# asmuth-archive/libsmatrix

Hardware: NVIDIA B200
Metric: incr_mops_c2 (higher is better)
Workload: dtype u32

## Files before the change

include/smatrix_b200.h:

```cpp
#ifndef SMATRIX_B200_H
#define SMATRIX_B200_H

#include "smatrix.h"

#ifdef __cplusplus
extern "C" {
#endif

smatrix_t* smatrix_b200_open(const char* fname, int device);
smatrix_t* smatrix_b200_open_arena(const char* fname, int device, size_t arena_bytes);

int   smatrix_b200_snapshot(smatrix_t* self);

int      smatrix_b200_snap_extent(smatrix_t* self, uint64_t* rows, uint64_t* bytes);
uint64_t smatrix_b200_snap_rows_base(uint64_t total_rows);
int      smatrix_b200_snap_layout(int fd, uint64_t total_rows, uint64_t total_bytes);
int      smatrix_b200_snap_write(smatrix_t* self, int fd, uint64_t byte_base, uint64_t first_entry);
int      smatrix_b200_snap_commit(const char* tmp, const char* fname);
typedef struct smx_loader_s smx_loader_t;
smx_loader_t* smatrix_b200_load_begin(smatrix_t* self, int fd, int share, int shares);
int  smatrix_b200_load_next(smx_loader_t* ld, const uint32_t** d_xs, const uint32_t** d_ys, const uint32_t** d_vs,
                            size_t* n_ops, const uint32_t** d_keys, const uint32_t** d_logs, size_t* n_rows);
void smatrix_b200_load_end(smx_loader_t* ld);
void smatrix_b200_load_fixup(smatrix_t* self, const uint32_t* d_keys, const uint32_t* d_logs, size_t n);
// ... 2 lines not shown
void* smatrix_b200_stream(smatrix_t* self);
void  smatrix_b200_sync(smatrix_t* self);

void  smatrix_b200_timer_start(smatrix_t* self);
float smatrix_b200_timer_stop_ms(smatrix_t* self);

enum {
  SMX_STAT_ROWS = 0,
  SMX_STAT_NNZ = 1,
  SMX_STAT_DIR_CAP = 2,
  SMX_STAT_SLAB_BYTES = 3,
  SMX_STAT_DEVICE_BYTES = 4,
  SMX_STAT_LAUNCHES = 5,
  SMX_STAT_ROUNDS = 6,
  SMX_STAT_ROW_GROWS = 7,
  SMX_STAT_DIR_GROWS = 8,
  SMX_STAT_KERNEL_NS = 9,
  SMX_STAT_NS_PARTITION = 10, SMX_STAT_NS_UPSERT = 11, SMX_STAT_NS_GROW_PLAN = 12,
  SMX_STAT_NS_SLAB = 13, SMX_STAT_NS_MIGRATE = 14, SMX_STAT_NS_DIR = 15,
  SMX_STAT_VALUE_SUM = 16,
  SMX_STAT_LIVE_BUCKET_BYTES = 17,
  SMX_STAT_FREE_BYTES = 18,
  SMX_STAT_RECYCLED = 19,
  SMX_STAT_H2D_BYTES = 20,
  SMX_STAT_D2H_BYTES = 21,
  SMX_STAT_BUCKET_BYTES = 22,
  SMX_STAT_SPILLED = 23,
  SMX_STAT_SLICED_GETS = 24,
  SMX_STAT_WIDE_CHUNKS = 25,
  SMX_STAT_NS_ALLOC = 26,
  SMX_STAT_ALLOCS = 27,
  SMX_STAT_TOPK_BIG = 28,
  SMX_STAT_TOPK_PASSES = 29,
  SMX_STAT_REC_BIG = 30
};
uint64_t smatrix_b200_stat(smatrix_t* self, int which);

void smatrix_b200_set_kernel_timing(smatrix_t* self, int on);

void smatrix_b200_set_get_slices(smatrix_t* self, int mode);

void* smatrix_b200_host_alloc(size_t bytes);
void  smatrix_b200_host_free(void* p);

void* smatrix_b200_dev_alloc(smatrix_t* self, size_t bytes);
void  smatrix_b200_dev_free(smatrix_t* self, void* p);
void  smatrix_b200_memcpy(smatrix_t* self, void* dst, const void* src, size_t bytes);
void  smatrix_b200_memset0(smatrix_t* self, void* d_dst, size_t bytes);

void smatrix_b200_gen_c2_ops(smatrix_t* self, uint64_t seed, uint64_t first, size_t count,
                             uint32_t rows, uint32_t ycols, uint32_t* d_xs, uint32_t* d_ys);
void smatrix_b200_gen_c2_queries(smatrix_t* self, uint64_t seed_get, uint64_t seed_build,
                                 uint64_t first, size_t count, uint64_t n_build, uint32_t rows,
                                 uint32_t ycols, uint32_t* d_xs, uint32_t* d_ys);

void smatrix_b200_gen_c3_ops(smatrix_t* self, uint64_t seed, uint64_t first, size_t count,
                             const uint64_t* d_thr, uint32_t items, uint32_t* d_xs, uint32_t* d_ys);
void smatrix_b200_gen_c3_queries(smatrix_t* self, uint64_t seed_get, uint64_t seed_build, uint64_t first,
                                 size_t count, uint64_t n_build, const uint64_t* d_thr, uint32_t items,
                                 uint32_t* d_xs, uint32_t* d_ys);
void smatrix_b200_gen_c4_lens(smatrix_t* self, uint64_t seed, uint64_t first, size_t count,
                              const uint64_t* d_thr, uint32_t kmax, uint32_t* d_lens);
void smatrix_b200_gen_c4_ops(smatrix_t* self, uint64_t seed, uint64_t first, size_t count,
                             const uint64_t* d_offs, uint32_t rows, uint32_t* d_xs, uint32_t* d_ys,
                             uint32_t* d_vs);

double smatrix_b200_probe_random_read(smatrix_t* self, size_t footprint_bytes, size_t accesses, int width);
// ... 47 lines not shown
```

libsmatrix_b200/binding.py:

```python
from __future__ import annotations

import ctypes as C
import os

HERE = os.path.dirname(os.path.abspath(__file__))
DEFAULT_SO = os.environ.get("SMATRIX_B200_LIB") or os.path.join(HERE, "lib", "libsmatrix_b200.so")

u32p = C.POINTER(C.c_uint32)
u64p = C.POINTER(C.c_uint64)

PROTOTYPES = {
    "smatrix_open": (C.c_void_p, [C.c_char_p]),
    "smatrix_close": (None, [C.c_void_p]),
    "smatrix_get": (C.c_uint32, [C.c_void_p, C.c_uint32, C.c_uint32]),
    "smatrix_set": (C.c_uint32, [C.c_void_p, C.c_uint32, C.c_uint32, C.c_uint32]),
    "smatrix_incr": (C.c_uint32, [C.c_void_p, C.c_uint32, C.c_uint32, C.c_uint32]),
    "smatrix_decr": (C.c_uint32, [C.c_void_p, C.c_uint32, C.c_uint32, C.c_uint32]),
    "smatrix_rowlen": (C.c_uint32, [C.c_void_p, C.c_uint32]),
    "smatrix_getrow": (C.c_uint32, [C.c_void_p, C.c_uint32, C.c_void_p, C.c_size_t]),
    "smatrix_incr_batch": (None, [C.c_void_p, C.c_void_p, C.c_void_p, C.c_void_p, C.c_size_t]),
    "smatrix_decr_batch": (None, [C.c_void_p, C.c_void_p, C.c_void_p, C.c_void_p, C.c_size_t]),
    "smatrix_set_batch": (None, [C.c_void_p, C.c_void_p, C.c_void_p, C.c_void_p, C.c_size_t]),
    "smatrix_incr_batch_out": (None, [C.c_void_p, C.c_void_p, C.c_void_p, C.c_void_p, C.c_size_t, C.c_void_p]),
    "smatrix_decr_batch_out": (None, [C.c_void_p, C.c_void_p, C.c_void_p, C.c_void_p, C.c_size_t, C.c_void_p]),
# ... 86 lines not shown
    "smatrix_b200_shard_close": (None, [C.c_void_p]),
    "smatrix_b200_shard_local": (C.c_void_p, [C.c_void_p]),
    "smatrix_b200_shard_rank": (C.c_int, [C.c_void_p]),
    "smatrix_b200_shard_world": (C.c_int, [C.c_void_p]),
    "smatrix_b200_shard_reserve": (None, [C.c_void_p, C.c_size_t, C.c_size_t]),
    "smatrix_b200_shard_incr_batch": (None, [C.c_void_p, C.c_void_p, C.c_void_p, C.c_void_p, C.c_size_t, C.c_int]),
    "smatrix_b200_shard_decr_batch": (None, [C.c_void_p, C.c_void_p, C.c_void_p, C.c_void_p, C.c_size_t, C.c_int]),
    "smatrix_b200_shard_set_batch": (None, [C.c_void_p, C.c_void_p, C.c_void_p, C.c_void_p, C.c_size_t]),
    "smatrix_b200_shard_incr_batch_out": (None, [C.c_void_p, C.c_void_p, C.c_void_p, C.c_void_p, C.c_size_t, C.c_void_p]),
    "smatrix_b200_shard_decr_batch_out": (None, [C.c_void_p, C.c_void_p, C.c_void_p, C.c_void_p, C.c_size_t, C.c_void_p]),
    "smatrix_b200_shard_set_batch_out": (None, [C.c_void_p, C.c_void_p, C.c_void_p, C.c_void_p, C.c_size_t, C.c_void_p]),
    "smatrix_b200_shard_get_batch": (None, [C.c_void_p, C.c_void_p, C.c_void_p, C.c_size_t, C.c_void_p]),
    "smatrix_b200_shard_rowlen_batch": (None, [C.c_void_p, C.c_void_p, C.c_size_t, C.c_void_p]),
    "smatrix_b200_shard_cf_neighbors_batch": (C.c_uint64, [C.c_void_p, C.c_void_p, C.c_size_t, C.c_void_p, C.c_void_p,
                                                          C.c_void_p, C.c_uint64]),
    "smatrix_b200_shard_cf_topk_batch": (None, [C.c_void_p, C.c_void_p, C.c_size_t, C.c_uint32, C.c_void_p,
                                                C.c_void_p, C.c_void_p]),
    "smatrix_b200_shard_cf_recommend_batch": (None, [C.c_void_p, C.c_void_p, C.c_void_p, C.c_size_t, C.c_uint32,
                                                     C.c_void_p, C.c_void_p, C.c_void_p]),
    "smatrix_b200_shard_getrow_batch": (C.c_uint64, [C.c_void_p, C.c_void_p, C.c_size_t, C.c_void_p, C.c_void_p,
                                                    C.c_uint64]),
    "smatrix_b200_shard_stat": (C.c_uint64, [C.c_void_p, C.c_int]),
    "smatrix_b200_shard_stat_reset": (None, [C.c_void_p]),
    "smatrix_b200_shard_barrier": (None, [C.c_void_p]),
    "smatrix_b200_shard_sum": (C.c_uint64, [C.c_void_p, C.c_uint64]),
    "smatrix_b200_shard_max": (C.c_uint64, [C.c_void_p, C.c_uint64]),
})

STAT = {"rows": 0, "nnz": 1, "dir_cap": 2, "slab_bytes": 3, "device_bytes": 4, "launches": 5,
        "rounds": 6, "row_grows": 7, "dir_grows": 8, "kernel_ns": 9, "ns_partition": 10, "ns_upsert": 11,
        "ns_grow_plan": 12, "ns_slab": 13, "ns_migrate": 14, "ns_dir": 15, "value_sum": 16,
        "live_bucket_bytes": 17, "free_bytes": 18, "recycled": 19, "h2d_bytes": 20, "d2h_bytes": 21, "bucket_bytes": 22, "spilled": 23,
        "sliced_gets": 24, "wide_chunks": 25, "ns_alloc": 26, "allocs": 27,
        "topk_big": 28, "topk_passes": 29, "rec_big": 30}

_cache: dict[str, C.CDLL] = {}


def load(path: str | None = None) -> C.CDLL:
    path = os.path.abspath(path or DEFAULT_SO)
    lib = _cache.get(path)
    if lib is None:
        if not os.path.exists(path):
            raise ImportError(
                f"{path} not found: build the CUDA library first "
                "(python -m libsmatrix_b200.build). There is no CPU fallback.")
        lib = C.CDLL(path)
        for name, (res, args) in PROTOTYPES.items():
            fn = getattr(lib, name)
            fn.restype = res
            fn.argtypes = args
        _cache[path] = lib
    return lib
```

libsmatrix_b200/csrc/smx_host.c:

```c
#define _GNU_SOURCE
#include <cuda_runtime_api.h>
#include <pthread.h>
#include <stdarg.h>
#include <stdio.h>
#include <stdlib.h>
#include <string.h>
#include <time.h>
#include <errno.h>
#include <fcntl.h>
#include <sys/stat.h>
#include <sys/types.h>
#include <unistd.h>

#include "../../include/smatrix.h"
#include "../../include/smatrix_b200.h"
#include "../../include/smatrix_batch.h"
#include "smx_internal.h"

#define SMX_DIR_LOG_DEFAULT 20u
#define SMX_CHUNK_DEFAULT (1u << 26)
#define SMX_STAGE_MAX (1u << 23)
#define SMX_SEG_MIN ((size_t)64 << 20)
#define SMX_SEG_MAX ((size_t)16 << 30)
#define SMX_MAX_ROUNDS 128
// ... 74 lines not shown
    smx_dbuf_t rows;
    smx_dbuf_t host_out;
    smx_dbuf_t spill;
    smx_dbuf_t bo_addr[2], bo_idx[2], bo_seg, bo_tiles, bo_out, bo_sort;
    smx_dbuf_t tk_ctl;
    smx_dbuf_t tk_off;
    smx_dbuf_t tk_big;
    smx_dbuf_t tk_cids, tk_cscores;
    smx_dbuf_t tk_ids, tk_scores;
    smx_dbuf_t rc_in, rc_pos, rc_ctl, rc_items, rc_sort, rc_tids, rc_tscores, rc_red, rc_rids, rc_rscores;
    smx_dbuf_t rc_big, rc_keys, rc_vals, rc_flags;
    smx_dbuf_t ld_raw, ld_tiles, ld_cnt, ld_off, ld_ops, ld_fix;
  } db;
  uint32_t topk_pairs;
  uint64_t n_topk_big, n_topk_passes;
  uint64_t n_rec_big;

  unsigned long long* free_ptr[SMX_CLASSES];
  uint32_t free_cap[SMX_CLASSES];
  int debug;
  int migrate_tiles;
  uint32_t spill_cap;
  uint64_t n_spilled;
  int recycle;
  int presize;
  int get_slices;
  int get_flags;
  uint32_t get_slice_min;
  uint64_t n_sliced_gets;
  uint64_t n_wide_chunks;
  double alloc_ns;
  uint64_t n_allocs;

  uint64_t n_launches, n_rounds, n_row_grows, n_dir_grows, n_recycled;
  uint64_t bucket_bytes;
  uint64_t h2d_bytes, d2h_bytes;
  double phase_ns[8];
  int timing;
  cudaEvent_t ev0, ev1, t_start, t_stop;
  double kernel_ns;
  int preagg;
  char* fname;
  uint32_t* snap_keys;
  uint64_t snap_rows;
  uint64_t* snap_hoff;
  uint32_t* snap_hkeys;
};

static void smx_die(const char* fmt, ...) {
  va_list ap;
  printf("libsmatrix error: ");
  va_start(ap, fmt);
  vprintf(fmt, ap);
  va_end(ap);
  printf("\n");
  fflush(stdout);
  abort();
}
#define CK(call)                                                                        \
  do {                                                                                  \
    cudaError_t e_ = (call);                                                            \
    if (e_ != cudaSuccess) smx_die("%s failed: %s (%s:%d)", #call, cudaGetErrorString(e_), \
                                   __FILE__, __LINE__);                                 \
  } while (0)

static uint32_t env_u32(const char* name, uint32_t dflt) {
  const char* v = getenv(name);
// ... 319 lines not shown
  if (!s->dir_in_arena) CK(cudaFree(s->dir));
  else slab_give_back(s, (char*)s->dir, (size_t)s->dir_cap * sizeof(smx_row_t));
  s->dir = nd;
  s->dir_in_arena = in_arena;
  s->dir_cap = new_cap;
  s->n_dir_grows++;
  s->phase_ns[PH_DIR] += now_ns() - t0;
  return 1;
}

static void zero_round_counters(smatrix_t* s) {
  CK(cudaMemsetAsync(&s->d_ctl->n_defer, 0,
                     offsetof(smx_ctl_t, scratch) - offsetof(smx_ctl_t, n_defer), s->stream));
}

static void run_pass(smatrix_t* s, smx_ops_t ops, int op, int pass, const uint32_t* list, uint32_t m) {
  int flip = 0;
  uint32_t prev_defer = 0xFFFFFFFFu;
  for (int round = 0; m > 0; round++) {
    if (round >= SMX_MAX_ROUNDS) smx_die("update pass does not converge (%u ops left)", m);
    double t0 = now_ns();
    const uint64_t used_before = s->h_ctl->dir_used;
    zero_round_counters(s);
    s->lists.defer_out = s->defer[flip];
    timed_begin(s);
    smx_launch_upsert(s->stream, view_of(s), ops, s->lists, op, pass, list, m, s->preagg);
    timed_end(s);
    s->n_launches++;
    s->n_rounds++;
    read_ctl(s);
    timed_collect(s);
    s->phase_ns[PH_UPSERT] += now_ns() - t0;
    const smx_ctl_t c = *s->h_ctl;
    if (c.n_grow) grow_rows(s, c.n_grow);
    if (c.n_defer == 0) break;
    if (c.n_dirfull) {
      const uint64_t accepted = (uint64_t)m - c.n_defer;
      const uint64_t created = c.dir_used > used_before ? c.dir_used - used_before : 0;
      double ratio = accepted ? (double)created / (double)accepted : 1.0;
      if (ratio > 1.0) ratio = 1.0;
      if (ratio < 0.05) ratio = 0.05;
      uint64_t need = 4 * (c.dir_used + (uint64_t)(ratio * (double)c.n_dirfull));
      uint64_t cap = pow2_at_least(need);
      if (cap < s->dir_cap * 2) cap = s->dir_cap * 2;
      if (cap > s->dir_cap * 64) cap = s->dir_cap * 64;
      resize_dir(s, cap, 0);
    } else if (!c.n_grow && c.n_defer >= prev_defer) {
      smx_die("update pass made no progress (%u ops deferred)", c.n_defer);
    }
    prev_defer = c.n_defer;
    list = s->defer[flip];
    m = c.n_defer;
    flip ^= 1;
  }
}

static void maybe_shrink_dir(smatrix_t* s) {
  const uint64_t used = s->h_ctl->dir_used;
  uint64_t fit = pow2_at_least(4 * (used ? used : 1));
  const uint64_t floor_cap = 1ull << s->dir_log_min;
  if (fit < floor_cap) fit = floor_cap;
  if (fit * 4 <= s->dir_cap && fit > s->shrink_refused) resize_dir(s, fit, 1);
}

static void slice_geometry(const smatrix_t* s, uint32_t* parts_log, uint32_t* shift) {
  uint32_t dir_log = 0;
// ... 1541 lines not shown
      CK(cudaMemsetAsync(&s->d_ctl->scratch, 0, 8, s->stream));
      CK(cudaMemsetAsync(d_cnt, 0, 4, s->stream));
      smx_launch_sum_values(s->stream, view_of(s), big, d_cnt);
      copy_d2h(s, &s->h_small->n_big_sums, d_cnt, 4, s->stream);
      CK(cudaStreamSynchronize(s->stream));
      smx_launch_sum_values_big(s->stream, view_of(s), big, s->h_small->n_big_sums);
      s->n_launches += 2;
      read_ctl(s);
      r = s->h_ctl->scratch;
      break;
    }
    case SMX_STAT_LIVE_BUCKET_BYTES:
      CK(cudaMemsetAsync(&s->d_ctl->scratch, 0, 8, s->stream));
      smx_launch_live_bytes(s->stream, view_of(s));
      s->n_launches++;
      read_ctl(s);
      r = s->h_ctl->scratch;
      break;
    case SMX_STAT_FREE_BYTES:
      read_ctl(s);
      for (uint32_t c = SMX_MIN_SLAB_LOG; c < SMX_CLASSES; c++)
        if (s->h_ctl->free_cnt[c] > 0) r += (uint64_t)s->h_ctl->free_cnt[c] * (8ull << c);
      break;
    case SMX_STAT_RECYCLED: r = s->n_recycled; break;
    case SMX_STAT_BUCKET_BYTES: r = s->bucket_bytes; break;
    case SMX_STAT_SPILLED: r = s->n_spilled; break;
    case SMX_STAT_SLICED_GETS: r = s->n_sliced_gets; break;
    case SMX_STAT_WIDE_CHUNKS: r = s->n_wide_chunks; break;
    case SMX_STAT_NS_ALLOC: r = (uint64_t)s->alloc_ns; break;
    case SMX_STAT_ALLOCS: r = s->n_allocs; break;
    case SMX_STAT_TOPK_BIG: r = s->n_topk_big; break;
    case SMX_STAT_TOPK_PASSES: r = s->n_topk_passes; break;
    case SMX_STAT_REC_BIG: r = s->n_rec_big; break;
    case SMX_STAT_H2D_BYTES: r = s->h2d_bytes; break;
    case SMX_STAT_D2H_BYTES: r = s->d2h_bytes; break;
    case SMX_STAT_DIR_CAP: r = s->dir_cap; break;
    case SMX_STAT_SLAB_BYTES: r = s->slab_bytes; break;
    case SMX_STAT_DEVICE_BYTES: {
      r = s->seg_bytes + s->dir_cap * sizeof(smx_row_t) + (uint64_t)s->list_cap * (6 * 4 + sizeof(smx_plan_t)) +
          (uint64_t)s->stage_cap * 24 + (uint64_t)s->addrs_cap * 8 + (uint64_t)s->part_cap * 16;
      const smx_dbuf_t* db = (const smx_dbuf_t*)&s->db;
      for (size_t b = 0; b < sizeof s->db / sizeof *db; b++) r += db[b].bytes;
      break;
    }
    case SMX_STAT_LAUNCHES: r = s->n_launches; break;
    case SMX_STAT_ROUNDS: r = s->n_rounds; break;
    case SMX_STAT_ROW_GROWS: r = s->n_row_grows; break;
    case SMX_STAT_DIR_GROWS: r = s->n_dir_grows; break;
    case SMX_STAT_KERNEL_NS: r = (uint64_t)s->kernel_ns; break;
    case SMX_STAT_NS_PARTITION: r = (uint64_t)s->phase_ns[PH_PARTITION]; break;
    case SMX_STAT_NS_UPSERT: r = (uint64_t)s->phase_ns[PH_UPSERT]; break;
    case SMX_STAT_NS_GROW_PLAN: r = (uint64_t)s->phase_ns[PH_GROW_PLAN]; break;
    case SMX_STAT_NS_SLAB: r = (uint64_t)s->phase_ns[PH_SLAB]; break;
    case SMX_STAT_NS_MIGRATE: r = (uint64_t)s->phase_ns[PH_MIGRATE]; break;
    case SMX_STAT_NS_DIR: r = (uint64_t)s->phase_ns[PH_DIR]; break;
    default: break;
  }
  leave(s);
  return r;
}

void* smatrix_b200_host_alloc(size_t bytes) {
  void* p = NULL;
  if (cudaHostAlloc(&p, bytes ? bytes : 1, cudaHostAllocDefault) != cudaSuccess) return NULL;
  return p;
}
// ... 310 lines not shown
```

libsmatrix_b200/csrc/smx_internal.h:

```cpp
#ifndef SMX_INTERNAL_H
#define SMX_INTERNAL_H

#include <stddef.h>
#include <stdint.h>

#ifdef __cplusplus
extern "C" {
#endif

#define SMX_META_CAPLOG 0x3Fu
#define SMX_META_USED   0x100u
#define SMX_META_ZC     0x200u
#define SMX_META_D      0x400u
#define SMX_META_SLOG_SHIFT 16
#define SMX_META_SLOG   (0x1Fu << SMX_META_SLOG_SHIFT)
#define SMX_META_T0P    0x800u
#define SMX_META_GROW   0x1000u
#define SMX_INLINE_LOG  2u
#define SMX_MIN_SLAB_LOG 4u
#define SMX_MAX_CAPLOG  31u
#define SMX_BIG_LOG     13u
#define SMX_MID_LOG     9u
#define SMX_ZERO_LOG    9u
#define SMX_CLASSES     32u
// ... 24 lines not shown
  uint32_t n_recycled;
  uint32_t n_spill;
  uint32_t dir_probe_max;
  unsigned long long plan_bytes;
  unsigned long long need_zero;
  uint32_t grow_from[SMX_CLASSES];
  unsigned long long scratch;
  int32_t free_cnt[SMX_CLASSES];
  unsigned long long* free_stack[SMX_CLASSES];
  uint32_t slice_used[SMX_DIR_SLICES];
} smx_ctl_t;

typedef struct {
  smx_row_t* dir;
  uint64_t dir_cap;
  uint32_t slice_shift;
  uint32_t slice_limit;
  smx_ctl_t* ctl;
} smx_view_t;

typedef struct {
  const uint32_t* xs;
  const uint32_t* ys;
  const uint32_t* vs;
  const uint32_t* idx;
  uint32_t v_const;
  uint32_t n;
} smx_ops_t;

typedef struct {
  uint32_t entry;
  uint32_t newlog;
  uint64_t off;
} smx_plan_t;

typedef struct {
  uint32_t* defer_out;
  uint32_t* late;
  uint32_t* grow;
  uint32_t* t0rows;
  smx_plan_t* plan;
  uint32_t* big;
  uint32_t* mid;
} smx_lists_t;

enum { SMX_OP_INCR = 0, SMX_OP_DECR = 1, SMX_OP_SETZERO = 2 };
enum { SMX_PASS_COL0 = 0, SMX_PASS_EARLY = 1, SMX_PASS_LATE = 2 };

typedef void* smx_stream_t;

void smx_launch_upsert(smx_stream_t stream, smx_view_t v, smx_ops_t ops, smx_lists_t l, int op,
                       int pass, const uint32_t* list, uint32_t m, int preaggregate);
void smx_launch_grow_plan(smx_stream_t stream, smx_view_t v, smx_lists_t l, uint32_t n_grow);
void smx_launch_free_push(smx_stream_t stream, smx_view_t v, smx_lists_t l, uint32_t n_grow);
void smx_launch_migrate(smx_stream_t stream, smx_view_t v, smx_lists_t l, uint32_t n_grow,
                        uint32_t n_mid, uint32_t n_big, void* region_base, int skip_big);
void smx_launch_migrate_tiles(smx_stream_t stream, smx_view_t v, smx_lists_t l, uint32_t n_big, void* region_base,
                              unsigned long long* spill, uint32_t spill_cap);
void smx_launch_migrate_tiles_finish(smx_stream_t stream, smx_view_t v, smx_lists_t l, uint32_t n_big, void* region_base,
                                     const unsigned long long* spill, uint32_t n_spill);
void smx_launch_sketch(smx_stream_t stream, const uint32_t* xs, uint32_t n, uint32_t* bitmap,
                       uint32_t bits_log, smx_ctl_t* ctl);
void smx_launch_live_bytes(smx_stream_t stream, smx_view_t v);
void smx_launch_dir_rehash(smx_stream_t stream, smx_view_t from, smx_view_t to);
void smx_launch_finalize_t0(smx_stream_t stream, smx_view_t v, const uint32_t* t0rows, uint32_t n);
void smx_launch_sync_rowlen(smx_stream_t stream, smx_view_t v, const uint32_t* rows, uint32_t n);
// ... 133 lines not shown
```

libsmatrix_b200/csrc/smx_kernels.cu:

```cuda
#include "smx_internal.h"

#ifdef SMX_HOSTSIM
#include "hostsim.h"
#include "cuda_runtime_api.h"
#include <algorithm>
#include <vector>
#else
#include <cuda_runtime.h>
#include <cub/device/device_radix_sort.cuh>
#define SMX_WARP 32
#define SMX_LAUNCH(kern, grid, block, stream, ...) \
  kern<<<(grid), (block), 0, (cudaStream_t)(stream)>>>(__VA_ARGS__)
#define SMX_ACTIVEMASK(key) __activemask()
#endif

typedef unsigned long long ull;
#define SMX_FULL 0xffffffffu
#if defined(SMX_HOSTSIM) && SMX_WARP == 1
#define SMX_BLOCK 1
#else
#define SMX_BLOCK (8 * SMX_WARP)
#endif

#define SCAN_PER_THREAD 8
// ... 189 lines not shown
      }
    }
  }
  return SLOT_FULL;
}

template <bool ONCE = false>
__device__ __forceinline__ uint32_t slot_find(const smx_row_t* e, const Hdr& h, uint32_t y,
                                              uint32_t** where) {
  const uint32_t caplog = h.meta & SMX_META_CAPLOG;
  const ull* base = (caplog == SMX_INLINE_LOG) ? (const ull*)e->inl : (const ull*)h.slots;
  const uint32_t nsec = 1u << (caplog - 2u);
  uint32_t s = smx_mix_col(y) & (nsec - 1u);
  for (uint32_t probe = 0; probe < nsec; ++probe, s = (s + 1u) & (nsec - 1u)) {
    const ull* sec = base + 4ull * s;
    ull c[4];
    if (ONCE) ld_sector_once(sec, c);
    else ld_sector(sec, c);
    bool hole = false;
#pragma unroll
    for (int k = 0; k < 4; ++k) {
      if ((uint32_t)c[k] == y) {
        if (where) *where = (uint32_t*)(sec + k) + 1;
        return (uint32_t)(c[k] >> 32);
      }
      hole |= (c[k] == 0ull);
    }
    if (hole) break;
  }
  if (where) *where = nullptr;
  return 0u;
}

template <int OP>
__device__ __forceinline__ int upsert_one(const smx_view_t& V, const smx_lists_t& S, int pass,
                                          uint32_t ord, uint32_t x, uint32_t y, uint32_t v) {
  smx_row_t* e;
  Hdr h;
  int r = dir_find(V, x, true, &e, &h);
  if (r == DIR_FULL) return ST_DIRFULL;
  if (pass == SMX_PASS_COL0) {
    apply_value<OP>(&e->c0, v);
    if (v != 0u && !(h.meta & SMX_META_ZC)) {
      atomicMax(&e->t0inv, ~ord);
      if (!(h.meta & SMX_META_T0P)) {
        uint32_t old = atomicOr(&e->meta, SMX_META_T0P);
        if (!(old & SMX_META_T0P)) S.t0rows[agg_inc(&V.ctl->n_t0)] = x;
      }
    }
    return ST_OK;
  }
  if (pass == SMX_PASS_EARLY && (h.meta & SMX_META_T0P)) {
    if (ord > ~h.t0inv) return ST_LATE;
  }
  const int r2 = slot_upsert<OP>(e, h, y, v);
  if (r2 == SLOT_DONE) return ST_OK;
  if (r2 == SLOT_FULL) atomicAdd(&e->want, 1u);
  if (!(h.meta & SMX_META_GROW)) {
    uint32_t old = atomicOr(&e->meta, SMX_META_GROW);
    if (!(old & SMX_META_GROW)) S.grow[agg_inc(&V.ctl->n_grow)] = (uint32_t)(e - V.dir);
  }
  return r2 == SLOT_FULL ? ST_DEFER : ST_OK;
}

#ifndef SMX_UPSERT_MIN_BLOCKS
#define SMX_UPSERT_MIN_BLOCKS 6
#endif
template <int OP>
__global__ void __launch_bounds__(SMX_BLOCK, SMX_UPSERT_MIN_BLOCKS)
k_upsert(smx_view_t V, smx_ops_t O, smx_lists_t S, int pass, const uint32_t* list, uint32_t m,
         int preagg) {
  __shared__ uint32_t s_defer[4 * SMX_BLOCK];
  __shared__ uint32_t s_ndefer, s_ndirfull, s_base;
  if (threadIdx.x == 0) { s_ndefer = 0u; s_ndirfull = 0u; }
  __syncthreads();
  const uint32_t lane = lane_id();
  const uint32_t stride = gridDim.x * blockDim.x;
  const uint32_t m_up = (m + (SMX_WARP - 1)) / SMX_WARP * SMX_WARP;
  for (uint32_t j = blockIdx.x * blockDim.x + threadIdx.x; j < m_up; j += stride) {
    bool act = j < m;
    uint32_t pos = 0, ord = 0, x = 0, y = 0, v = 0;
    if (act) {
      pos = list ? list[j] : j;
      ord = O.idx ? O.idx[pos] : pos;
      x = O.xs[pos];
      y = O.ys[pos];
      v = O.vs ? O.vs[pos] : O.v_const;
      if (!list) act = (pass == SMX_PASS_COL0) ? (y == 0u) : (y != 0u);
    }
    bool lead = act;
    uint32_t vsum = v;
    unsigned peers = 1u << lane;
    int leader = (int)lane;
    if (preagg) {
      const ull k64 = ((ull)x << 32) | (ull)y;
      const unsigned valid = __ballot_sync(SMX_FULL, act);
      peers = __match_any_sync(SMX_FULL, k64) & valid;
      const bool dup = act && (peers != (1u << lane));
      if (__any_sync(SMX_FULL, dup)) {
        vsum = 0u;
        uint32_t best = 0xFFFFFFFFu, best_nz = 0xFFFFFFFFu;
        int leader_nz = -1;
        for (int src = 0; src < SMX_WARP; ++src) {
          const uint32_t tv = __shfl_sync(SMX_FULL, v, src);
          const uint32_t to = __shfl_sync(SMX_FULL, ord, src);
          if ((peers >> src) & 1u) {
            vsum += tv;
            if (to < best) { best = to; leader = src; }
            if (tv != 0u && to < best_nz) { best_nz = to; leader_nz = src; }
          }
        }
        if (pass == SMX_PASS_COL0 && leader_nz >= 0) leader = leader_nz;
        if (OP == SMX_OP_SETZERO && pass == SMX_PASS_COL0) vsum = leader_nz >= 0 ? 1u : 0u;
        lead = act && (leader == (int)lane);
      }
    }
    int status = ST_OK;
    if (lead) status = upsert_one<OP>(V, S, pass, ord, x, y, vsum);
    if (preagg) {
      __syncwarp();
      const int ls = __shfl_sync(SMX_FULL, status, act ? leader : (int)lane);
      if (act && !lead) status = ls;
    }
    if (act && (status == ST_DEFER || status == ST_DIRFULL)) {
      const uint32_t k = atomicAdd(&s_ndefer, 1u);
      if (k < 4u * SMX_BLOCK) s_defer[k] = pos;
      else S.defer_out[agg_inc(&V.ctl->n_defer)] = pos;
      if (status == ST_DIRFULL) atomicAdd(&s_ndirfull, 1u);
    } else if (act && status == ST_LATE) {
      S.late[agg_inc(&V.ctl->n_late)] = pos;
    }
  }
  __syncthreads();
  const uint32_t nd = s_ndefer < 4u * SMX_BLOCK ? s_ndefer : 4u * SMX_BLOCK;
  if (threadIdx.x == 0 && nd) {
    s_base = atomicAdd(&V.ctl->n_defer, nd);
    if (s_ndirfull) atomicAdd(&V.ctl->n_dirfull, s_ndirfull);
  }
  __syncthreads();
  for (uint32_t k = threadIdx.x; k < nd; k += blockDim.x) S.defer_out[s_base + k] = s_defer[k];
}

#define SMX_SMEM_MIGRATE_LOG 8u
#define SMX_MID_SMEM_LOG 12u

__global__ void __launch_bounds__(SMX_BLOCK)
k_grow_plan(smx_view_t V, smx_lists_t S, uint32_t n_grow) {
  const uint32_t lane = lane_id();
  const uint32_t stride = gridDim.x * blockDim.x;
  const uint32_t n_up = (n_grow + (SMX_WARP - 1)) / SMX_WARP * SMX_WARP;
  for (uint32_t j = blockIdx.x * blockDim.x + threadIdx.x; j < n_up; j += stride) {
    const bool act = j < n_grow;
    ull bytes = 0, recycled = 0;
    uint32_t entry = 0, newlog = 0, caplog = 0;
    if (act) {
      entry = S.grow[j];
      Hdr h = ld_hdr(V.dir + entry);
      caplog = h.meta & SMX_META_CAPLOG;
      const ull need = 2ull * ((ull)h.live + (ull)h.want);
      newlog = caplog + (caplog < 8u ? 3u : (caplog >= SMX_MID_LOG ? 2u : 1u));
      if (newlog > 8u && caplog < 8u) newlog = 8u;
      if (newlog < SMX_MIN_SLAB_LOG) newlog = SMX_MIN_SLAB_LOG;
      while ((1ull << newlog) < need && newlog < SMX_MAX_CAPLOG) ++newlog;
      {
        const unsigned grp = __match_any_sync(SMX_ACTIVEMASK(0), newlog);
        const int leader = __ffs(grp) - 1;
        const int cnt = __popc(grp), rank = __popc(grp & ((1u << lane) - 1u));
        int base = 0;
        if ((int)lane == leader) {
          base = atomicSub(&V.ctl->free_cnt[newlog], cnt);
          if (base < cnt) atomicAdd(&V.ctl->free_cnt[newlog], cnt - (base > 0 ? base : 0));
        }
        base = __shfl_sync(grp, base, leader);
        const int at = base - 1 - rank;
        if (at >= 0) recycled = (ull)V.ctl->free_stack[newlog][at];
      }
      bytes = recycled ? 0ull : (8ull << newlog);
      if (caplog > SMX_INLINE_LOG) {
        const unsigned grp = __match_any_sync(SMX_ACTIVEMASK(0), caplog);
        if ((int)lane == __ffs(grp) - 1) atomicAdd(&V.ctl->grow_from[caplog], (uint32_t)__popc(grp));
      }
    }
    ull incl = bytes;
    for (uint32_t d = 1; d < SMX_WARP; d <<= 1) {
      ull t = __shfl_up_sync(SMX_FULL, incl, d);
      if (lane >= d) incl += t;
    }
    const ull total = __shfl_sync(SMX_FULL, incl, SMX_WARP - 1);
    ull base = 0;
    if (lane == 0 && total) base = atomicAdd(&V.ctl->plan_bytes, total);
    base = __shfl_sync(SMX_FULL, base, 0);
    if (act) {
      smx_plan_t p;
      p.entry = entry;
      p.newlog = newlog;
      p.off = recycled ? (SMX_PLAN_RECYCLED | recycled) : (base + incl - bytes);
      S.plan[j] = p;
      if (recycled) agg_inc(&V.ctl->n_recycled);
      const bool by_grid = caplog >= SMX_BIG_LOG || (caplog >= SMX_MID_LOG && newlog > SMX_MID_SMEM_LOG);
      if (by_grid) S.big[agg_inc(&V.ctl->n_big)] = j;
      else if (caplog >= SMX_MID_LOG) S.mid[agg_inc(&V.ctl->n_mid)] = j;
      const bool in_place = by_grid || (caplog < SMX_MID_LOG && newlog > SMX_SMEM_MIGRATE_LOG);
      if (in_place && !recycled) agg_inc64(&V.ctl->need_zero);
    }
  }
}

__global__ void __launch_bounds__(SMX_BLOCK)
k_free_push(smx_view_t V, smx_lists_t S, uint32_t n_grow) {
  const uint32_t lane = lane_id();
  for (uint32_t j = blockIdx.x * blockDim.x + threadIdx.x; j < n_grow; j += gridDim.x * blockDim.x) {
    const Hdr h = ld_hdr(V.dir + S.plan[j].entry);
    const uint32_t caplog = h.meta & SMX_META_CAPLOG;
    if (caplog <= SMX_INLINE_LOG) continue;
    const unsigned grp = __match_any_sync(SMX_ACTIVEMASK(0), caplog);
    const int leader = __ffs(grp) - 1;
    int base = 0;
    if ((int)lane == leader) base = atomicAdd(&V.ctl->free_cnt[caplog], __popc(grp));
    base = __shfl_sync(grp, base, leader);
    V.ctl->free_stack[caplog][base + __popc(grp & ((1u << lane) - 1u))] = h.slots;
  }
}

__device__ __forceinline__ void place_cell(ull* base, uint32_t caplog, ull cell) {
  const uint32_t nsec = 1u << (caplog - 2u);
  uint32_t s = smx_mix_col((uint32_t)cell) & (nsec - 1u);
  for (uint32_t probe = 0; probe < nsec; ++probe, s = (s + 1u) & (nsec - 1u)) {
    ull* sec = base + 4ull * s;
    ull c[4];
    ld_sector(sec, c);
#pragma unroll
    for (int k = 0; k < 4; ++k) {
      if (c[k] != 0ull) continue;
      if (atomicCAS(sec + k, 0ull, cell) == 0ull) return;
    }
  }
}
__device__ __forceinline__ void place_cell_smem(ull* sb, uint32_t nsec, ull c) {
  uint32_t sidx = smx_mix_col((uint32_t)c) & (nsec - 1u);
  for (bool placed = false; !placed; sidx = (sidx + 1u) & (nsec - 1u))
    for (int k = 0; k < 4 && !placed; ++k)
      placed = (atomicCAS(&sb[4u * sidx + k], 0ull, c) == 0ull);
}

__device__ __forceinline__ ull* plan_bucket(const smx_plan_t& p, char* region) {
  return (p.off & SMX_PLAN_RECYCLED) ? (ull*)(p.off & ~SMX_PLAN_RECYCLED) : (ull*)(region + p.off);
}

__device__ __forceinline__ void finish_growth(smx_row_t* e, const Hdr& h, ull* nb, uint32_t newlog) {
  e->slots = (ull)nb;
  e->want = 0u;
  e->meta = (h.meta & ~(SMX_META_CAPLOG | SMX_META_GROW)) | newlog;
}

__global__ void __launch_bounds__(SMX_BLOCK)
k_migrate(smx_view_t V, smx_lists_t S, uint32_t n_grow, char* region) {
  __shared__ ull sbuf[SMX_BLOCK / SMX_WARP][1u << SMX_SMEM_MIGRATE_LOG];
  const uint32_t lane = lane_id();
  const uint32_t wib = threadIdx.x / SMX_WARP;
  const uint32_t warp = (blockIdx.x * blockDim.x + threadIdx.x) / SMX_WARP;
  const uint32_t nwarps = gridDim.x * blockDim.x / SMX_WARP;
  for (uint32_t j = warp; j < n_grow; j += nwarps) {
    const smx_plan_t p = S.plan[j];
    smx_row_t* e = V.dir + p.entry;
    const Hdr h = ld_hdr(e);
    const uint32_t caplog = h.meta & SMX_META_CAPLOG;
    if (caplog >= SMX_MID_LOG) continue;
    ull* ob = (caplog == SMX_INLINE_LOG) ? (ull*)e->inl : (ull*)h.slots;
    ull* nb = plan_bucket(p, region);
    const uint32_t cap = 1u << caplog;
    if (p.newlog <= SMX_SMEM_MIGRATE_LOG) {
      ull* sb = sbuf[wib];
      const uint32_t ncap = 1u << p.newlog, nsec = ncap >> 2;
      for (uint32_t i = lane; i < ncap; i += SMX_WARP) sb[i] = 0ull;
      __syncwarp();
      for (uint32_t s0 = lane; s0 < cap; s0 += SMX_WARP) {
        const ull c = ob[s0];
        if (c != 0ull) place_cell_smem(sb, nsec, c);
      }
      __syncwarp();
      for (uint32_t i = lane; i < ncap; i += SMX_WARP) nb[i] = sb[i];
    } else {
      for (uint32_t s0 = lane; s0 < cap; s0 += SMX_WARP) {
        const ull c = ob[s0];
        if (c != 0ull) place_cell(nb, p.newlog, c);
      }
    }
    __syncwarp();
    if (lane == 0) finish_growth(e, h, nb, p.newlog);
  }
}

__global__ void __launch_bounds__(SMX_BLOCK)
k_migrate_mid(smx_view_t V, smx_lists_t S, uint32_t n_mid, char* region) {
  __shared__ ull sb[1u << SMX_MID_SMEM_LOG];
  for (uint32_t j = blockIdx.x; j < n_mid; j += gridDim.x) {
    const smx_plan_t p = S.plan[S.mid[j]];
    smx_row_t* e = V.dir + p.entry;
    const Hdr h = ld_hdr(e);
    const uint32_t caplog = h.meta & SMX_META_CAPLOG;
    ull* ob = (ull*)h.slots;
    ull* nb = plan_bucket(p, region);
    const uint32_t cap = 1u << caplog;
    {
      const uint32_t ncap = 1u << p.newlog, nsec = ncap >> 2;
      for (uint32_t i = threadIdx.x; i < ncap; i += blockDim.x) sb[i] = 0ull;
      __syncthreads();
      for (uint32_t s0 = threadIdx.x; s0 < cap; s0 += blockDim.x) {
        const ull c = ob[s0];
        ob[s0] = 0ull;
        if (c != 0ull) place_cell_smem(sb, nsec, c);
      }
      __syncthreads();
      for (uint32_t i = threadIdx.x; i < ncap; i += blockDim.x) nb[i] = sb[i];
    }
    __syncthreads();
    if (threadIdx.x == 0) finish_growth(e, h, nb, p.newlog);
    __syncthreads();
  }
}

__global__ void __launch_bounds__(SMX_BLOCK)
k_migrate_big(smx_view_t V, smx_lists_t S, uint32_t big_first, char* region) {
  const smx_plan_t p = S.plan[S.big[big_first + blockIdx.y]];
  smx_row_t* e = V.dir + p.entry;
  const Hdr h = ld_hdr(e);
  const uint32_t caplog = h.meta & SMX_META_CAPLOG;
  ull* ob = (ull*)h.slots;
  ull* nb = plan_bucket(p, region);
  const ull cap = 1ull << caplog;
  for (ull s = blockIdx.x * blockDim.x + threadIdx.x; s < cap; s += (ull)gridDim.x * blockDim.x) {
    const ull c = ob[s];
    ob[s] = 0ull;
    if (c != 0ull) place_cell(nb, p.newlog, c);
  }
}
__global__ void k_migrate_big_finish(smx_view_t V, smx_lists_t S, uint32_t n_big, char* region) {
  for (uint32_t b = blockIdx.x * blockDim.x + threadIdx.x; b < n_big; b += gridDim.x * blockDim.x) {
    const smx_plan_t p = S.plan[S.big[b]];
    smx_row_t* e = V.dir + p.entry;
    const Hdr h = ld_hdr(e);
    finish_growth(e, h, plan_bucket(p, region), p.newlog);
  }
}

#ifndef MIG_TILE_LOG
#define MIG_TILE_LOG 10u
#endif
#define MIG_TILE (1u << MIG_TILE_LOG)
__device__ __forceinline__ bool sector_is_full(const ull* sec) {
  ull c[4];
  ld_sector(sec, c);
  return c[0] != 0ull && c[1] != 0ull && c[2] != 0ull && c[3] != 0ull;
}
__device__ __forceinline__ void tile_take_sector(const ull* sec, ull* sm, uint32_t t0, uint32_t n_new, uint32_t j,
                                                 smx_ctl_t* ctl, ull* spill, uint32_t spill_cap) {
  ull c[4];
  ld_sector(sec, c);
#pragma unroll
  for (int k = 0; k < 4; ++k) {
    if (c[k] == 0ull) continue;
    const uint32_t hn = smx_mix_col((uint32_t)c[k]) & (n_new - 1u);
    if (hn - t0 >= MIG_TILE) continue;
    bool placed = false;
    for (uint32_t q = hn - t0; q < MIG_TILE && !placed; ++q)
      for (int w = 0; w < 4 && !placed; ++w) placed = (atomicCAS(&sm[4u * q + w], 0ull, c[k]) == 0ull);
    if (!placed) {
      const uint32_t at = atomicAdd(&ctl->n_spill, 1u);
      if (at < spill_cap) { spill[2ull * at] = (ull)j; spill[2ull * at + 1] = c[k]; }
    }
  }
}
__global__ void __launch_bounds__(SMX_BLOCK)
k_migrate_tiles(smx_view_t V, smx_lists_t S, uint32_t big_first, char* region, ull* spill, uint32_t spill_cap) {
  __shared__ ull sm[4u * MIG_TILE];
// ... 1584 lines not shown
extern "C" void smx_launch_upsert(smx_stream_t st, smx_view_t v, smx_ops_t ops, smx_lists_t l,
                                  int op, int pass, const uint32_t* list, uint32_t m,
                                  int preaggregate) {
  if (m == 0) return;
  ull want_blocks = ((ull)m + 4ull * SMX_BLOCK - 1) / (4ull * SMX_BLOCK);
  if (want_blocks < 1) want_blocks = 1;
  const uint32_t grid = (uint32_t)want_blocks;
  const int pre = (preaggregate && !list && pass != SMX_PASS_LATE && SMX_WARP > 1) ? 1 : 0;
  if (op == SMX_OP_INCR) {
    auto k = k_upsert<SMX_OP_INCR>;
    SMX_LAUNCH(k, grid, SMX_BLOCK, st, v, ops, l, pass, list, m, pre);
  } else if (op == SMX_OP_DECR) {
    auto k = k_upsert<SMX_OP_DECR>;
    SMX_LAUNCH(k, grid, SMX_BLOCK, st, v, ops, l, pass, list, m, pre);
  } else {
    auto k = k_upsert<SMX_OP_SETZERO>;
    SMX_LAUNCH(k, grid, SMX_BLOCK, st, v, ops, l, pass, list, m, pre);
  }
}

extern "C" void smx_launch_grow_plan(smx_stream_t st, smx_view_t v, smx_lists_t l, uint32_t n_grow) {
  if (!n_grow) return;
  SMX_LAUNCH(k_grow_plan, grid_for(n_grow), SMX_BLOCK, st, v, l, n_grow);
}

extern "C" void smx_launch_free_push(smx_stream_t st, smx_view_t v, smx_lists_t l, uint32_t n_grow) {
  if (!n_grow) return;
  SMX_LAUNCH(k_free_push, grid_for(n_grow), SMX_BLOCK, st, v, l, n_grow);
}

extern "C" void smx_launch_migrate(smx_stream_t st, smx_view_t v, smx_lists_t l, uint32_t n_grow,
                                   uint32_t n_mid, uint32_t n_big, void* region, int skip_big) {
  if (!n_grow) return;
  if (n_grow > n_mid + n_big)
    SMX_LAUNCH(k_migrate, grid_for((ull)n_grow * SMX_WARP), SMX_BLOCK, st, v, l, n_grow, (char*)region);
  if (n_mid) {
    const uint32_t cap = (uint32_t)smx_grid_blocks();
    SMX_LAUNCH(k_migrate_mid, n_mid < cap ? n_mid : cap, SMX_BLOCK, st, v, l, n_mid, (char*)region);
  }
  if (skip_big) return;
  for (uint32_t first = 0; first < n_big; first += 32768u) {
    const uint32_t cnt = (n_big - first < 32768u) ? n_big - first : 32768u;
    dim3 grid(SMX_WARP > 1 ? 64u : 2u, cnt, 1u);
    SMX_LAUNCH(k_migrate_big, grid, SMX_BLOCK, st, v, l, first, (char*)region);
  }
  if (n_big) SMX_LAUNCH(k_migrate_big_finish, grid_for(n_big), SMX_BLOCK, st, v, l, n_big, (char*)region);
}

extern "C" void smx_launch_migrate_tiles(smx_stream_t st, smx_view_t v, smx_lists_t l, uint32_t n_big, void* region,
                                         unsigned long long* spill, uint32_t spill_cap) {
  for (uint32_t first = 0; first < n_big; first += 32768u) {
    const uint32_t cnt = (n_big - first < 32768u) ? n_big - first : 32768u;
    dim3 grid(SMX_WARP > 1 ? 32u : 2u, cnt, 1u);
    SMX_LAUNCH(k_migrate_tiles, grid, SMX_BLOCK, st, v, l, first, (char*)region, (ull*)spill, spill_cap);
  }
}
extern "C" void smx_launch_migrate_tiles_finish(smx_stream_t st, smx_view_t v, smx_lists_t l, uint32_t n_big, void* region,
                                                const unsigned long long* spill, uint32_t n_spill) {
  if (n_spill) SMX_LAUNCH(k_spill_insert, grid_for(n_spill), SMX_BLOCK, st, v, l, (char*)region, (const ull*)spill, n_spill);
  for (uint32_t first = 0; first < n_big; first += 32768u) {
    const uint32_t cnt = (n_big - first < 32768u) ? n_big - first : 32768u;
    dim3 grid(SMX_WARP > 1 ? 32u : 2u, cnt, 1u);
    SMX_LAUNCH(k_zero_old_big, grid, SMX_BLOCK, st, v, l, first);
  }
  if (n_big) SMX_LAUNCH(k_migrate_big_finish, grid_for(n_big), SMX_BLOCK, st, v, l, n_big, (char*)region);
}
extern "C" void smx_launch_sketch(smx_stream_t st, const uint32_t* xs, uint32_t n, uint32_t* bitmap,
                                  uint32_t bits_log, smx_ctl_t* ctl) {
// ... 479 lines not shown
```

Measured before the change: 13200.

## Batch grow-list appends in shared memory and prefetch old cells in migrate

Upsert now buffers grow-row entries in shared memory and flushes them with one global atomic per block instead of one per row. The grow plan records the old slot pointer and meta, so migrate and free_push no longer reread the directory header. k_migrate becomes a persistent, grid-capped kernel in which each warp loads a batch of plans with one lane per plan. It prefetches the first old cells of upcoming rows a few iterations ahead to hide gather latency. The shared migrate buffer also grows to 2^9 cells per warp, which raises shared memory use, and a deferred-ops stat is added.

```diff
diff --git a/include/smatrix_b200.h b/include/smatrix_b200.h
--- a/include/smatrix_b200.h
+++ b/include/smatrix_b200.h
@@ -58,7 +58,8 @@
   SMX_STAT_ALLOCS = 27,
   SMX_STAT_TOPK_BIG = 28,
   SMX_STAT_TOPK_PASSES = 29,
-  SMX_STAT_REC_BIG = 30
+  SMX_STAT_REC_BIG = 30,
+  SMX_STAT_DEFERRED_OPS = 31
 };
 uint64_t smatrix_b200_stat(smatrix_t* self, int which);
 
diff --git a/libsmatrix_b200/binding.py b/libsmatrix_b200/binding.py
--- a/libsmatrix_b200/binding.py
+++ b/libsmatrix_b200/binding.py
@@ -142,7 +142,7 @@
         "ns_grow_plan": 12, "ns_slab": 13, "ns_migrate": 14, "ns_dir": 15, "value_sum": 16,
         "live_bucket_bytes": 17, "free_bytes": 18, "recycled": 19, "h2d_bytes": 20, "d2h_bytes": 21, "bucket_bytes": 22, "spilled": 23,
         "sliced_gets": 24, "wide_chunks": 25, "ns_alloc": 26, "allocs": 27,
-        "topk_big": 28, "topk_passes": 29, "rec_big": 30}
+        "topk_big": 28, "topk_passes": 29, "rec_big": 30, "deferred_ops": 31}
 
 _cache: dict[str, C.CDLL] = {}
 
diff --git a/libsmatrix_b200/csrc/smx_host.c b/libsmatrix_b200/csrc/smx_host.c
--- a/libsmatrix_b200/csrc/smx_host.c
+++ b/libsmatrix_b200/csrc/smx_host.c
@@ -130,7 +130,7 @@
   double alloc_ns;
   uint64_t n_allocs;
 
-  uint64_t n_launches, n_rounds, n_row_grows, n_dir_grows, n_recycled;
+  uint64_t n_launches, n_rounds, n_row_grows, n_dir_grows, n_recycled, n_deferred;
   uint64_t bucket_bytes;
   uint64_t h2d_bytes, d2h_bytes;
   double phase_ns[8];
@@ -516,6 +516,7 @@
     timed_collect(s);
     s->phase_ns[PH_UPSERT] += now_ns() - t0;
     const smx_ctl_t c = *s->h_ctl;
+    s->n_deferred += c.n_defer;
     if (c.n_grow) grow_rows(s, c.n_grow);
     if (c.n_defer == 0) break;
     if (c.n_dirfull) {
@@ -2123,6 +2124,7 @@
     case SMX_STAT_TOPK_BIG: r = s->n_topk_big; break;
     case SMX_STAT_TOPK_PASSES: r = s->n_topk_passes; break;
     case SMX_STAT_REC_BIG: r = s->n_rec_big; break;
+    case SMX_STAT_DEFERRED_OPS: r = s->n_deferred; break;
     case SMX_STAT_H2D_BYTES: r = s->h2d_bytes; break;
     case SMX_STAT_D2H_BYTES: r = s->d2h_bytes; break;
     case SMX_STAT_DIR_CAP: r = s->dir_cap; break;
diff --git a/libsmatrix_b200/csrc/smx_internal.h b/libsmatrix_b200/csrc/smx_internal.h
--- a/libsmatrix_b200/csrc/smx_internal.h
+++ b/libsmatrix_b200/csrc/smx_internal.h
@@ -80,6 +80,9 @@
   uint32_t entry;
   uint32_t newlog;
   uint64_t off;
+  uint64_t old;
+  uint32_t meta;
+  uint32_t pad;
 } smx_plan_t;
 
 typedef struct {
diff --git a/libsmatrix_b200/csrc/smx_kernels.cu b/libsmatrix_b200/csrc/smx_kernels.cu
--- a/libsmatrix_b200/csrc/smx_kernels.cu
+++ b/libsmatrix_b200/csrc/smx_kernels.cu
@@ -245,9 +245,10 @@
   return 0u;
 }
 
+#define SMX_NO_GROW 0xFFFFFFFFu
 template <int OP>
-__device__ __forceinline__ int upsert_one(const smx_view_t& V, const smx_lists_t& S, int pass,
-                                          uint32_t ord, uint32_t x, uint32_t y, uint32_t v) {
+__device__ __forceinline__ int upsert_one(const smx_view_t& V, int pass, uint32_t ord, uint32_t x, uint32_t y,
+                                          uint32_t v, uint32_t* t0rows, uint32_t* grow) {
   smx_row_t* e;
   Hdr h;
   int r = dir_find(V, x, true, &e, &h);
@@ -258,7 +259,7 @@
       atomicMax(&e->t0inv, ~ord);
       if (!(h.meta & SMX_META_T0P)) {
         uint32_t old = atomicOr(&e->meta, SMX_META_T0P);
-        if (!(old & SMX_META_T0P)) S.t0rows[agg_inc(&V.ctl->n_t0)] = x;
+        if (!(old & SMX_META_T0P)) t0rows[agg_inc(&V.ctl->n_t0)] = x;
       }
     }
     return ST_OK;
@@ -271,7 +272,7 @@
   if (r2 == SLOT_FULL) atomicAdd(&e->want, 1u);
   if (!(h.meta & SMX_META_GROW)) {
     uint32_t old = atomicOr(&e->meta, SMX_META_GROW);
-    if (!(old & SMX_META_GROW)) S.grow[agg_inc(&V.ctl->n_grow)] = (uint32_t)(e - V.dir);
+    if (!(old & SMX_META_GROW)) *grow = (uint32_t)(e - V.dir);
   }
   return r2 == SLOT_FULL ? ST_DEFER : ST_OK;
 }
@@ -283,9 +284,9 @@
 __global__ void __launch_bounds__(SMX_BLOCK, SMX_UPSERT_MIN_BLOCKS)
 k_upsert(smx_view_t V, smx_ops_t O, smx_lists_t S, int pass, const uint32_t* list, uint32_t m,
          int preagg) {
-  __shared__ uint32_t s_defer[4 * SMX_BLOCK];
-  __shared__ uint32_t s_ndefer, s_ndirfull, s_base;
-  if (threadIdx.x == 0) { s_ndefer = 0u; s_ndirfull = 0u; }
+  __shared__ uint32_t s_defer[4 * SMX_BLOCK], s_grow[4 * SMX_BLOCK];
+  __shared__ uint32_t s_ndefer, s_ndirfull, s_ngrow, s_base, s_gbase;
+  if (threadIdx.x == 0) { s_ndefer = 0u; s_ndirfull = 0u; s_ngrow = 0u; }
   __syncthreads();
   const uint32_t lane = lane_id();
   const uint32_t stride = gridDim.x * blockDim.x;
@@ -329,7 +330,13 @@
       }
     }
     int status = ST_OK;
-    if (lead) status = upsert_one<OP>(V, S, pass, ord, x, y, vsum);
+    uint32_t grow = SMX_NO_GROW;
+    if (lead) status = upsert_one<OP>(V, pass, ord, x, y, vsum, S.t0rows, &grow);
+    if (grow != SMX_NO_GROW) {
+      const uint32_t k = atomicAdd(&s_ngrow, 1u);
+      if (k < 4u * SMX_BLOCK) s_grow[k] = grow;
+      else S.grow[agg_inc(&V.ctl->n_grow)] = grow;
+    }
     if (preagg) {
       __syncwarp();
       const int ls = __shfl_sync(SMX_FULL, status, act ? leader : (int)lane);
@@ -346,15 +353,18 @@
   }
   __syncthreads();
   const uint32_t nd = s_ndefer < 4u * SMX_BLOCK ? s_ndefer : 4u * SMX_BLOCK;
-  if (threadIdx.x == 0 && nd) {
-    s_base = atomicAdd(&V.ctl->n_defer, nd);
+  const uint32_t ng = s_ngrow < 4u * SMX_BLOCK ? s_ngrow : 4u * SMX_BLOCK;
+  if (threadIdx.x == 0) {
+    if (nd) s_base = atomicAdd(&V.ctl->n_defer, nd);
     if (s_ndirfull) atomicAdd(&V.ctl->n_dirfull, s_ndirfull);
+    if (ng) s_gbase = atomicAdd(&V.ctl->n_grow, ng);
   }
   __syncthreads();
   for (uint32_t k = threadIdx.x; k < nd; k += blockDim.x) S.defer_out[s_base + k] = s_defer[k];
-}
-
-#define SMX_SMEM_MIGRATE_LOG 8u
+  for (uint32_t k = threadIdx.x; k < ng; k += blockDim.x) S.grow[s_gbase + k] = s_grow[k];
+}
+
+#define SMX_SMEM_MIGRATE_LOG 9u
 #define SMX_MID_SMEM_LOG 12u
 
 __global__ void __launch_bounds__(SMX_BLOCK)
@@ -366,9 +376,10 @@
     const bool act = j < n_grow;
     ull bytes = 0, recycled = 0;
     uint32_t entry = 0, newlog = 0, caplog = 0;
+    Hdr h;
     if (act) {
       entry = S.grow[j];
-      Hdr h = ld_hdr(V.dir + entry);
+      h = ld_hdr(V.dir + entry);
       caplog = h.meta & SMX_META_CAPLOG;
       const ull need = 2ull * ((ull)h.live + (ull)h.want);
       newlog = caplog + (caplog < 8u ? 3u : (caplog >= SMX_MID_LOG ? 2u : 1u));
@@ -408,6 +419,9 @@
       p.entry = entry;
       p.newlog = newlog;
       p.off = recycled ? (SMX_PLAN_RECYCLED | recycled) : (base + incl - bytes);
+      p.old = h.slots;
+      p.meta = h.meta;
+      p.pad = 0u;
       S.plan[j] = p;
       if (recycled) agg_inc(&V.ctl->n_recycled);
       const bool by_grid = caplog >= SMX_BIG_LOG || (caplog >= SMX_MID_LOG && newlog > SMX_MID_SMEM_LOG);
@@ -423,15 +437,15 @@
 k_free_push(smx_view_t V, smx_lists_t S, uint32_t n_grow) {
   const uint32_t lane = lane_id();
   for (uint32_t j = blockIdx.x * blockDim.x + threadIdx.x; j < n_grow; j += gridDim.x * blockDim.x) {
-    const Hdr h = ld_hdr(V.dir + S.plan[j].entry);
-    const uint32_t caplog = h.meta & SMX_META_CAPLOG;
+    const smx_plan_t p = S.plan[j];
+    const uint32_t caplog = p.meta & SMX_META_CAPLOG;
     if (caplog <= SMX_INLINE_LOG) continue;
     const unsigned grp = __match_any_sync(SMX_ACTIVEMASK(0), caplog);
     const int leader = __ffs(grp) - 1;
     int base = 0;
     if ((int)lane == leader) base = atomicAdd(&V.ctl->free_cnt[caplog], __popc(grp));
     base = __shfl_sync(grp, base, leader);
-    V.ctl->free_stack[caplog][base + __popc(grp & ((1u << lane) - 1u))] = h.slots;
+    V.ctl->free_stack[caplog][base + __popc(grp & ((1u << lane) - 1u))] = p.old;
   }
 }
 
@@ -456,51 +470,85 @@
       placed = (atomicCAS(&sb[4u * sidx + k], 0ull, c) == 0ull);
 }
 
-__device__ __forceinline__ ull* plan_bucket(const smx_plan_t& p, char* region) {
-  return (p.off & SMX_PLAN_RECYCLED) ? (ull*)(p.off & ~SMX_PLAN_RECYCLED) : (ull*)(region + p.off);
-}
-
-__device__ __forceinline__ void finish_growth(smx_row_t* e, const Hdr& h, ull* nb, uint32_t newlog) {
+__device__ __forceinline__ ull* bucket_at(ull off, char* region) {
+  return (off & SMX_PLAN_RECYCLED) ? (ull*)(off & ~SMX_PLAN_RECYCLED) : (ull*)(region + off);
+}
+__device__ __forceinline__ ull* plan_bucket(const smx_plan_t& p, char* region) { return bucket_at(p.off, region); }
+
+__device__ __forceinline__ void finish_growth(smx_row_t* e, uint32_t meta, ull* nb, uint32_t newlog) {
   e->slots = (ull)nb;
   e->want = 0u;
-  e->meta = (h.meta & ~(SMX_META_CAPLOG | SMX_META_GROW)) | newlog;
-}
-
-__global__ void __launch_bounds__(SMX_BLOCK)
+  e->meta = (meta & ~(SMX_META_CAPLOG | SMX_META_GROW)) | newlog;
+}
+
+__device__ __forceinline__ ull old_cell(const smx_view_t& V, uint32_t entry, uint32_t meta, ull old, uint32_t i) {
+  const uint32_t caplog = meta & SMX_META_CAPLOG;
+  if (caplog >= SMX_MID_LOG || i >= (1u << caplog)) return 0ull;
+  return caplog == SMX_INLINE_LOG ? V.dir[entry].inl[i] : ((const ull*)old)[i];
+}
+
+#define MIG_AHEAD 3
+#define MIG_BLOCKS_PER_SM 6
+__global__ void __launch_bounds__(SMX_BLOCK, MIG_BLOCKS_PER_SM)
 k_migrate(smx_view_t V, smx_lists_t S, uint32_t n_grow, char* region) {
   __shared__ ull sbuf[SMX_BLOCK / SMX_WARP][1u << SMX_SMEM_MIGRATE_LOG];
   const uint32_t lane = lane_id();
-  const uint32_t wib = threadIdx.x / SMX_WARP;
-  const uint32_t warp = (blockIdx.x * blockDim.x + threadIdx.x) / SMX_WARP;
-  const uint32_t nwarps = gridDim.x * blockDim.x / SMX_WARP;
-  for (uint32_t j = warp; j < n_grow; j += nwarps) {
-    const smx_plan_t p = S.plan[j];
-    smx_row_t* e = V.dir + p.entry;
-    const Hdr h = ld_hdr(e);
-    const uint32_t caplog = h.meta & SMX_META_CAPLOG;
-    if (caplog >= SMX_MID_LOG) continue;
-    ull* ob = (caplog == SMX_INLINE_LOG) ? (ull*)e->inl : (ull*)h.slots;
-    ull* nb = plan_bucket(p, region);
-    const uint32_t cap = 1u << caplog;
-    if (p.newlog <= SMX_SMEM_MIGRATE_LOG) {
-      ull* sb = sbuf[wib];
-      const uint32_t ncap = 1u << p.newlog, nsec = ncap >> 2;
-      for (uint32_t i = lane; i < ncap; i += SMX_WARP) sb[i] = 0ull;
-      __syncwarp();
-      for (uint32_t s0 = lane; s0 < cap; s0 += SMX_WARP) {
-        const ull c = ob[s0];
-        if (c != 0ull) place_cell_smem(sb, nsec, c);
+  ull* sb = sbuf[threadIdx.x / SMX_WARP];
+  const ull warp = (blockIdx.x * (ull)blockDim.x + threadIdx.x) / SMX_WARP;
+  const ull nwarps = (ull)gridDim.x * blockDim.x / SMX_WARP;
+  for (ull i0 = 0; warp + i0 * nwarps < n_grow; i0 += SMX_WARP) {
+    const ull jl = warp + (i0 + lane) * nwarps;
+    smx_plan_t mp;
+    mp.entry = 0u; mp.newlog = 0u; mp.off = 0ull; mp.old = 0ull; mp.meta = SMX_MID_LOG; mp.pad = 0u;
+    if (jl < n_grow) mp = S.plan[jl];
+    const uint32_t cnt = __popc(__ballot_sync(SMX_FULL, jl < n_grow));
+    ull ahead[MIG_AHEAD + 1];
+#pragma unroll
+    for (uint32_t d = 0; d < MIG_AHEAD; ++d) {
+      const uint32_t src = d < cnt ? d : 0u;
+      const uint32_t en = __shfl_sync(SMX_FULL, mp.entry, src), me = __shfl_sync(SMX_FULL, mp.meta, src);
+      const ull ol = __shfl_sync(SMX_FULL, mp.old, src);
+      ahead[d] = d < cnt ? old_cell(V, en, me, ol, lane) : 0ull;
+    }
+    for (uint32_t r = 0; r < cnt; ++r) {
+      {
+        const uint32_t nx = r + MIG_AHEAD, src = nx < cnt ? nx : 0u;
+        const uint32_t en = __shfl_sync(SMX_FULL, mp.entry, src), me = __shfl_sync(SMX_FULL, mp.meta, src);
+        const ull ol = __shfl_sync(SMX_FULL, mp.old, src);
+        ahead[MIG_AHEAD] = nx < cnt ? old_cell(V, en, me, ol, lane) : 0ull;
       }
-      __syncwarp();
-      for (uint32_t i = lane; i < ncap; i += SMX_WARP) nb[i] = sb[i];
-    } else {
-      for (uint32_t s0 = lane; s0 < cap; s0 += SMX_WARP) {
-        const ull c = ob[s0];
-        if (c != 0ull) place_cell(nb, p.newlog, c);
+      const uint32_t entry = __shfl_sync(SMX_FULL, mp.entry, r), meta = __shfl_sync(SMX_FULL, mp.meta, r);
+      const uint32_t newlog = __shfl_sync(SMX_FULL, mp.newlog, r);
+      const ull old = __shfl_sync(SMX_FULL, mp.old, r), off = __shfl_sync(SMX_FULL, mp.off, r);
+      const uint32_t caplog = meta & SMX_META_CAPLOG;
+      if (caplog < SMX_MID_LOG) {
+        ull* nb = bucket_at(off, region);
+        const ull* ob = caplog == SMX_INLINE_LOG ? (const ull*)V.dir[entry].inl : (const ull*)old;
+        const uint32_t cap = 1u << caplog;
+        if (newlog <= SMX_SMEM_MIGRATE_LOG) {
+          const uint32_t ncap = 1u << newlog, nsec = ncap >> 2;
+          for (uint32_t i = lane; i < ncap; i += SMX_WARP) sb[i] = 0ull;
+          __syncwarp();
+          if (ahead[0] != 0ull) place_cell_smem(sb, nsec, ahead[0]);
+          for (uint32_t s0 = lane + SMX_WARP; s0 < cap; s0 += SMX_WARP) {
+            const ull c = ob[s0];
+            if (c != 0ull) place_cell_smem(sb, nsec, c);
+          }
+          __syncwarp();
+          for (uint32_t i = lane; i < ncap; i += SMX_WARP) nb[i] = sb[i];
+        } else {
+          if (ahead[0] != 0ull) place_cell(nb, newlog, ahead[0]);
+          for (uint32_t s0 = lane + SMX_WARP; s0 < cap; s0 += SMX_WARP) {
+            const ull c = ob[s0];
+            if (c != 0ull) place_cell(nb, newlog, c);
+          }
+        }
+        __syncwarp();
+        if (lane == 0) finish_growth(V.dir + entry, meta, nb, newlog);
       }
-    }
-    __syncwarp();
-    if (lane == 0) finish_growth(e, h, nb, p.newlog);
+#pragma unroll
+      for (uint32_t d = 0; d < MIG_AHEAD; ++d) ahead[d] = ahead[d + 1];
+    }
   }
 }
 
@@ -528,7 +576,7 @@
       for (uint32_t i = threadIdx.x; i < ncap; i += blockDim.x) nb[i] = sb[i];
     }
     __syncthreads();
-    if (threadIdx.x == 0) finish_growth(e, h, nb, p.newlog);
+    if (threadIdx.x == 0) finish_growth(e, h.meta, nb, p.newlog);
     __syncthreads();
   }
 }
@@ -553,7 +601,7 @@
     const smx_plan_t p = S.plan[S.big[b]];
     smx_row_t* e = V.dir + p.entry;
     const Hdr h = ld_hdr(e);
-    finish_growth(e, h, plan_bucket(p, region), p.newlog);
+    finish_growth(e, h.meta, plan_bucket(p, region), p.newlog);
   }
 }
 
@@ -2204,8 +2252,10 @@
 extern "C" void smx_launch_migrate(smx_stream_t st, smx_view_t v, smx_lists_t l, uint32_t n_grow,
                                    uint32_t n_mid, uint32_t n_big, void* region, int skip_big) {
   if (!n_grow) return;
-  if (n_grow > n_mid + n_big)
-    SMX_LAUNCH(k_migrate, grid_for((ull)n_grow * SMX_WARP), SMX_BLOCK, st, v, l, n_grow, (char*)region);
+  if (n_grow > n_mid + n_big) {
+    const uint32_t cap = (uint32_t)smx_grid_blocks() / 8u * MIG_BLOCKS_PER_SM, want = grid_for((ull)n_grow * SMX_WARP);
+    SMX_LAUNCH(k_migrate, want < cap ? want : cap, SMX_BLOCK, st, v, l, n_grow, (char*)region);
+  }
   if (n_mid) {
     const uint32_t cap = (uint32_t)smx_grid_blocks();
     SMX_LAUNCH(k_migrate_mid, n_mid < cap ? n_mid : cap, SMX_BLOCK, st, v, l, n_mid, (char*)region);
```

Result: faster. 13500, median of 6 (+2.3%).
